# MayDomine/Burst-Attention

Hardware: AMD Instinct MI355X
Metric: attention_fwd_TFLOPs_per_GPU (higher is better)
Workload: dtype fp16; 1 GPU; b=1 seq=262144 h=32 d=128 non-causal; parallelism=ring sequence parallel, sp1

## Files before the change

### burst_attn_amd/build_ext.py

```python

import os
import subprocess
import sys
import sysconfig

PKG_DIR = os.path.dirname(os.path.abspath(__file__))
CSRC = os.path.join(PKG_DIR, "csrc")
BUILD = os.path.join(PKG_DIR, "csrc", "_build")
ARCH = os.environ.get("PYTORCH_ROCM_ARCH", "gfx950")
HIPCC = os.environ.get("HIPCC", "/opt/rocm/bin/hipcc")

DEVICE_SOURCES = ["attn_fwd.hip", "attn_bwd.hip", "probes.hip"]
HOST_SOURCES = ["ext_torch.cpp"]


def _run(cmd, verbose):
    if verbose:
        print("+ " + " ".join(cmd), flush=True)
    r = subprocess.run(cmd, capture_output=True, text=True)
    if r.returncode != 0:
        sys.stderr.write(r.stdout + r.stderr)
        raise RuntimeError(f"build command failed: {' '.join(cmd[:3])} ...")
    return r

# ... 63 lines not shown

def _build_asm_hsaco(verbose, force):
    import json
    import re

    src = os.path.join(CSRC, "attn_fwd.hip")
    s_path = os.path.join(BUILD, "attn_fwd_scaffold.s")
    o_path = os.path.join(BUILD, "attn_fwd_scaffold.o")
    hsaco = os.path.join(PKG_DIR, "_asm_fwd.hsaco")
    syms = os.path.join(PKG_DIR, "_asm_fwd_syms.json")
    patch_mod = os.path.join(PKG_DIR, "..", "tools", "s_patch.py")
    if not (force or _newer(src, hsaco) or _newer(patch_mod, hsaco)):
        return hsaco
    _run([HIPCC, f"--offload-arch={ARCH}", "-O3", "-std=c++17", "-DNDEBUG",
          "-S", "--cuda-device-only", src, "-o", s_path], verbose)
    clang = os.path.join(LLVM, "clang")
    lld = os.path.join(LLVM, "ld.lld")
    _run([clang, "-x", "assembler", "-target", "amdgcn-amd-amdhsa",
          f"-mcpu={ARCH}", "-c", s_path, "-o", o_path], verbose)
    _run([lld, "-shared", o_path, "-o", hsaco], verbose)
    text = open(s_path).read()
    names = {}
    for key, pat in (
        ("f16_accum", r"_ZN12_GLOBAL__N_115attn_fwd_kernelIDF16_Li128ELi64ELi1ELi0ELi1ELi512ELi2ELi0E\S*"),
        ("bf16_accum", r"_ZN12_GLOBAL__N_115attn_fwd_kernelIDF16bLi128ELi64ELi1ELi0ELi1ELi512ELi2ELi0E\S*"),
    ):
        m = re.search(r"\.globl\t(" + pat + ")", text)
        if m:
            names[key] = m.group(1)
    with open(syms, "w") as f:
        json.dump(names, f, indent=1)
    import importlib.util

    spec = importlib.util.spec_from_file_location("s_patch", patch_mod)
    s_patch = importlib.util.module_from_spec(spec)
    spec.loader.exec_module(s_patch)
    sp_path = os.path.join(BUILD, "attn_fwd_patched.s")
    spo_path = os.path.join(BUILD, "attn_fwd_patched.o")
    hsaco_p = os.path.join(PKG_DIR, "_asm_fwd_p.hsaco")
    s_patch.apply("qk_split", s_path, sp_path, list(names.values()))
    _run([clang, "-x", "assembler", "-target", "amdgcn-amd-amdhsa",
          f"-mcpu={ARCH}", "-c", sp_path, "-o", spo_path], verbose)
    _run([lld, "-shared", spo_path, "-o", hsaco_p], verbose)
    if verbose:
        print(f"built {hsaco} and {hsaco_p} (qk_split)")
    return hsaco


# ... 3 lines not shown
```

### burst_attn_amd/csrc/attn_common.h

```cpp
#pragma once
#include <hip/hip_runtime.h>
#include <stdint.h>

typedef __attribute__((ext_vector_type(8))) __bf16 bf16x8_t;
typedef __attribute__((ext_vector_type(8))) _Float16 f16x8_t;
typedef __attribute__((ext_vector_type(16))) float f32x16_t;
typedef __attribute__((ext_vector_type(2))) int i32x2_t;
typedef __attribute__((ext_vector_type(4))) unsigned int u32x4_t;

__device__ __forceinline__ float ba_exp2(float x) {
  return __builtin_amdgcn_exp2f(x);
}

#define BA_LOG2E 1.44269504088896340736f
#define BA_LN2 0.69314718055994530942f
#define BA_NEG_BIG (-1e30f)

template <typename T>
struct mfma_traits;

template <>
struct mfma_traits<_Float16> {
  using frag = f16x8_t;
  static __device__ __forceinline__ f32x16_t mma(frag a, frag b, f32x16_t c) {
// ... 30 lines not shown
template <int SWZ, int SWZ2 = 0>
__device__ __forceinline__ int ba_swz(int byte, int row) {
  return byte ^ ((((row & SWZ) ^ ((row >> 3) & SWZ2))) << 4);
}

template <typename T>
__device__ __forceinline__ void ba_build_frag_pair(
    const f32x16_t& p, typename mfma_traits<T>::frag out[2]) {
  using MT = mfma_traits<T>;
#pragma unroll
  for (int u = 0; u < 2; ++u) {
    unsigned int a0 = MT::pack2(p[8 * u + 0], p[8 * u + 1]);
    unsigned int a1 = MT::pack2(p[8 * u + 2], p[8 * u + 3]);
    unsigned int b0 = MT::pack2(p[8 * u + 4], p[8 * u + 5]);
    unsigned int b1 = MT::pack2(p[8 * u + 6], p[8 * u + 7]);
    i32x2_t r0 = __builtin_amdgcn_permlane32_swap((int)a0, (int)b0, false, false);
    i32x2_t r1 = __builtin_amdgcn_permlane32_swap((int)a1, (int)b1, false, false);
    u32x4_t w = {(unsigned int)r0[0], (unsigned int)r1[0],
                 (unsigned int)r0[1], (unsigned int)r1[1]};
    out[u] = __builtin_bit_cast(typename mfma_traits<T>::frag, w);
  }
}

__device__ __forceinline__ float ba_max16(const f32x16_t& v) {
  float a = fmaxf(fmaxf(v[0], v[1]), v[2]);
  float b = fmaxf(fmaxf(v[3], v[4]), v[5]);
  float c = fmaxf(fmaxf(v[6], v[7]), v[8]);
  float d = fmaxf(fmaxf(v[9], v[10]), v[11]);
  float e = fmaxf(fmaxf(v[12], v[13]), v[14]);
  float f = fmaxf(fmaxf(a, b), v[15]);
  return fmaxf(fmaxf(fmaxf(c, d), e), f);
}

template <typename T, int RS, int SWZ, int SWZ2 = 0>
__device__ __forceinline__ typename mfma_traits<T>::frag ba_ld_rowslice(
    const T* lds, int row, int elem0) {
  int byte = ba_swz<SWZ, SWZ2>(row * (2 * RS) + 2 * elem0, row);
  u32x4_t wv = *(const u32x4_t*)((const char*)lds + byte);
  return __builtin_bit_cast(typename mfma_traits<T>::frag, wv);
}

template <typename T, int RS_T, int SWZ_T, int SWZ2_T = 7>
__device__ __forceinline__ void ba_st_transposed(T* lds, int src_row, int d0,
                                                 const u32x4_t& chunk) {
  const T* e = (const T*)&chunk;
#pragma unroll
// ... 45 lines not shown
```

### burst_attn_amd/csrc/attn_fwd.hip

```cpp

#include "attn_common.h"
#include "attn_host.h"
#include "fwd_variants.h"
#include "gqa_heads.h"

#include <stddef.h>

namespace {

template <int N>
struct ba_ic {
  static constexpr int value = N;
};
struct ba_dyn {
  int value;
};
template <int N>
__device__ __forceinline__ int ba_buf_of(ba_ic<N>) { return N; }
__device__ __forceinline__ int ba_buf_of(ba_dyn d) { return d.value; }

template <typename T, int D, int KVBLK, int OUT_STATE, int VPATH, int SUBT,
          int NT = 512, int NBUF = 2, int KREG = 0>
__global__ __launch_bounds__(NT) void attn_fwd_kernel(
    const T* __restrict__ q, const T* __restrict__ k, const T* __restrict__ v,
    float* __restrict__ o, float* __restrict__ lse,
    int Sq, int Sk, int N, int G,
    int64_t q_sb, int64_t q_ss, int64_t q_sh,
    int64_t k_sb, int64_t k_ss, int64_t k_sh,
    int64_t v_sb, int64_t v_ss, int64_t v_sh,
    float scale, int causal,
    float* __restrict__ st_acc, float* __restrict__ st_m,
    float* __restrict__ st_l,
    int64_t a_sb, int64_t a_ss, int64_t a_sh,
    int64_t ml_sb, int64_t ml_sh, int carry_in) {
  using MT = mfma_traits<T>;
  using frag = typename MT::frag;
  constexpr int SWZ_K = (D == 128) ? 15 : 7;
  constexpr int SWZ_V = 7;
  constexpr int PT = (KVBLK * D / 8) / NT;
  constexpr int QROWS = NT / 2;
  static_assert(PT >= 1, "tile must fill at least one chunk per thread");

  static_assert(KREG != 1 || (SUBT == 1 && NBUF == 2 && VPATH == 0),
                "KREG=1 path: SUBT=1, NBUF=2, V^T image only");
  static_assert(KREG != 2 || (SUBT == 1 && NBUF == 4 && VPATH == 0),
                "KREG=2 path: SUBT=1, NBUF=4 (cross-barrier prefetch)");
  constexpr int IMGS_F = (KREG == 1) ? 1 : 2;
  __shared__ T lds[NBUF * IMGS_F * KVBLK * D];
  auto ldsK = [&](int buf) -> T* { return lds + buf * (IMGS_F * KVBLK * D); };
  auto ldsVT = [&](int buf) -> T* {
    return lds + buf * (IMGS_F * KVBLK * D) + (KREG == 1 ? 0 : KVBLK * D);
  };

  const int tid = threadIdx.x;
  const int lane = tid & 63;
  const int wave = tid >> 6;
  const int l31 = lane & 31;
  const int hi = lane >> 5;
  const int n = blockIdx.y;
  const int b = blockIdx.z;
  const int qb = blockIdx.x * QROWS + wave * 32;
  const int q_row = qb + l31;

  const T* qp = q + (int64_t)b * q_sb + (int64_t)n * q_sh;
  const int nkv = n / G;
  const T* kp = k + (int64_t)b * k_sb + (int64_t)nkv * k_sh;
  const T* vp = v + (int64_t)b * v_sb + (int64_t)nkv * v_sh;

  frag qf[D / 16];
// ... 47 lines not shown
  };
  auto qk_regs = [&](const frag* kf) BA_STEP {
    f32x16_t s = (f32x16_t)(0.f);
#pragma unroll
    for (int i = 0; i < D / 16; ++i) s = MT::mma(kf[i], qf[i], s);
    return s;
  };
  auto qk_lds = [&](int buf, int kvs) BA_STEP {
    f32x16_t s = (f32x16_t)(0.f);
#pragma unroll
    for (int i = 0; i < D / 16; ++i)
      s = MT::mma(k_frag(buf, kvs, i), qf[i], s);
    return s;
  };
  auto mask_sub = [&](f32x16_t& s, int base, int off) BA_STEP {
#pragma unroll
    for (int r = 0; r < 16; ++r) {
      const int kv_g = base + off + ba_crow(r, 0) + 4 * hi;
      if (!(kv_g < Sk && (!causal || kv_g <= q_row))) s[r] = BA_NEG_BIG;
    }
  };
  auto row_max2 = [&](const f32x16_t& s) BA_STEP {
    float tm = ba_max16(s);
    tm = fmaxf(tm, __shfl_xor(tm, 32));
    return tm * c2;
  };
  constexpr float DEFER_THR = 8.f;
  auto rescale = [&](float tm) BA_STEP {
    if (!__all(tm - m2 <= DEFER_THR)) {
      const float mnew = fmaxf(m2, tm);
      const float alpha = ba_exp2(m2 - mnew);
      m2 = mnew;
      lsum *= alpha;
#pragma unroll
      for (int dt = 0; dt < D / 32; ++dt)
#pragma unroll
        for (int r = 0; r < 16; ++r) ot[dt][r] *= alpha;
    }
  };
  auto softmax_tail = [&](f32x16_t& s, float tm, frag* pf) BA_STEP {
    rescale(tm);
    float rowsum = 0.f;
#pragma unroll
    for (int r = 0; r < 16; ++r) {
      s[r] = ba_exp2(__builtin_fmaf(s[r], c2, -m2));
      rowsum += s[r];
    }
    rowsum += __shfl_xor(rowsum, 32);
    lsum += rowsum;
    ba_build_frag_pair<T>(s, pf);
  };
  auto v_frag = [&](int buf, int drow, int kvc) BA_STEP -> frag {
    if (VPATH == 0)
      return ba_ld_rowslice<T, KVBLK, SWZ_V, 7>(ldsVT(buf), drow, kvc + 8 * hi);
    return ba_ld_tr16_frag<T, D>(ldsVT(buf), lane, kvc, drow & ~31);
  };
  auto pv_regs = [&](const frag* vv, const frag* pf) BA_STEP {
#pragma unroll
    for (int dt = 0; dt < D / 32; ++dt)
#pragma unroll
      for (int u = 0; u < 2; ++u)
        ot[dt] = MT::mma(vv[dt * 2 + u], pf[u], ot[dt]);
  };
  struct chunk_rc {
    int row, col8;
  };
  auto stage_rc = [&](int c) BA_STEP {
    const int flat = tid + c * NT;
    return chunk_rc{flat / (D / 8), flat % (D / 8)};
  };
#undef BA_STEP
// ... 39 lines not shown
    if (steady || v_kv0 >= 0) pv_regs(vvP, pvf);
    if (steady || p_kv0 >= 0) {
      softmax_tail(stP, tm, pvf);
      v_kv0 = p_kv0;
      const int kvs_l = (p_kv0 / 32) & 1;
#pragma unroll
      for (int dt = 0; dt < D / 32; ++dt)
#pragma unroll
        for (int u = 0; u < 2; ++u)
          vvP[dt * 2 + u] = v_frag(p_cur, dt * 32 + l31, kvs_l * 32 + 16 * u);
    }
    push_scores(stQ, t * KVBLK + kvs * 32, cur3, full);
  };

  uint32_t k_loff[PT], v_loff[PT];
#pragma unroll
  for (int c = 0; c < PT; ++c) {
    const auto [row, col8] = stage_rc(c);
    k_loff[c] = (uint32_t)((row * k_ss + col8 * 8) * (int64_t)sizeof(T));
    v_loff[c] = (uint32_t)((row * v_ss + col8 * 8) * (int64_t)sizeof(T));
  }
  const bool stage_lin =
      (int64_t)(KVBLK - 1) * k_ss * (int64_t)sizeof(T) + 16 <= 0xffffffffLL &&
      (int64_t)(KVBLK - 1) * v_ss * (int64_t)sizeof(T) + 16 <= 0xffffffffLL;
  auto issue_loads = [&](int tile, u32x4_t* kreg, u32x4_t* vreg) {
    const int kv0 = tile * KVBLK;
    if (SUBT == 1 && stage_lin && kv0 + KVBLK <= Sk) {
      const char* kb = (const char*)(kp + (int64_t)kv0 * k_ss);
      const char* vb = (const char*)(vp + (int64_t)kv0 * v_ss);
#pragma unroll
      for (int c = 0; c < PT; ++c) {
        if (KREG != 1) kreg[c] = *(const u32x4_t*)(kb + k_loff[c]);
        vreg[c] = *(const u32x4_t*)(vb + v_loff[c]);
      }
      return;
    }
#pragma unroll
    for (int c = 0; c < PT; ++c) {
      const auto [row, col8] = stage_rc(c);
      const int kvg = kv0 + row;
      const int kvc = kvg < Sk ? kvg : (Sk - 1);
      if (KREG != 1)
        kreg[c] = *(const u32x4_t*)(kp + (int64_t)kvc * k_ss + col8 * 8);
      vreg[c] = *(const u32x4_t*)(vp + (int64_t)kvc * v_ss + col8 * 8);
    }
  };
  auto write_lds = [&](int buf, const u32x4_t* kreg, const u32x4_t* vreg) {
#pragma unroll
    for (int c = 0; c < PT; ++c) {
      const auto [row, col8] = stage_rc(c);
      if (KREG != 1) {
        const int byte = ba_swz<SWZ_K>(row * (2 * D) + col8 * 16, row);
        *(u32x4_t*)((char*)ldsK(buf) + byte) = kreg[c];
      }
      if (VPATH == 0)
        ba_st_transposed<T, KVBLK, SWZ_V, 7>(ldsVT(buf), row, col8 * 8, vreg[c]);
      else
        ba_st_tr16row<T, D>(ldsVT(buf), row, col8 * 8, vreg[c]);
    }
  };
  auto load_k_sub = [&](int tile, int kvs, frag* dst) {
#pragma unroll
    for (int s = 0; s < D / 16; ++s) {
      const int kvg = tile * KVBLK + kvs * 32 + l31;
      const int kvc = kvg < Sk ? kvg : (Sk - 1);
      dst[s] = __builtin_bit_cast(
          frag, *(const u32x4_t*)(kp + (int64_t)kvc * k_ss + 16 * s + 8 * hi));
    }
  };

  frag kfr[KREG == 1 ? 2 : 1][D / 16];
  {
    u32x4_t kreg[PT], vreg[PT];
    issue_loads(0, kreg, vreg);
    write_lds(0, kreg, vreg);
    if (KREG == 1) {
      load_k_sub(0, 0, kfr[0]);
      load_k_sub(0, 1, kfr[KREG == 1 ? 1 : 0]);
// ... 169 lines not shown
    const float* __restrict__ acc, const float* __restrict__ m,
    const float* __restrict__ l, T* __restrict__ o, float* __restrict__ lse,
    int S, int N) {
  const int lane = threadIdx.x & 63;
  const int wave = threadIdx.x >> 6;
  constexpr int LPR = D / 16;
  const int rows_per_wave = 64 / LPR;
  const int row_in = wave * rows_per_wave + lane / LPR;
  const int sub = lane % LPR;
  const int s = blockIdx.x * 4 * rows_per_wave + row_in;
  const int n = blockIdx.y, b = blockIdx.z;
  if (s >= S) return;
  const float lv = l[((int64_t)b * N + n) * S + s];
  const float inv_l = 1.f / lv;
  const float* arow = acc + (((int64_t)b * S + s) * N + n) * D + sub * 16;
  T* orow = o + (((int64_t)b * S + s) * N + n) * D + sub * 16;
#pragma unroll
  for (int j = 0; j < 16; ++j) orow[j] = (T)(arow[j] * inv_l);
  if (sub == 0)
    lse[((int64_t)b * N + n) * S + s] =
        BA_LN2 * (m[((int64_t)b * N + n) * S + s] + log2f(lv));
}

}

extern "C" const char* bahip_last_error(void) { return ba_g_err; }

struct fwd_args {
  const void *q, *k, *v;
  float *o, *lse;
  int Sq, Sk, N, G;
  int64_t q_sb, q_ss, q_sh, k_sb, k_ss, k_sh, v_sb, v_ss, v_sh;
  float scale;
  int causal;
  float *st_acc, *st_m, *st_l;
  int64_t a_sb, a_ss, a_sh, ml_sb, ml_sh;
  int carry_in;
};

using production_kernel_t = decltype(&attn_fwd_kernel<
    _Float16, 128, 64, 1, BA_FWD_PRODUCTION.vpath, BA_FWD_PRODUCTION.subt,
    BA_FWD_PRODUCTION.nt, BA_FWD_PRODUCTION.nbuf, BA_FWD_PRODUCTION.kreg>);
static_assert(offsetof(fwd_args, carry_in) + sizeof(int) ==
                      kernarg_size<production_kernel_t>::value &&
                  sizeof(fwd_args) ==
                      (kernarg_size<production_kernel_t>::value + 7) / 8 * 8,
              "fwd_args must mirror attn_fwd_kernel's parameter list");

static dim3 fwd_grid(const fwd_args& a, int64_t B, int nt) {
  return dim3((unsigned)((a.Sq + nt / 2 - 1) / (nt / 2)), (unsigned)a.N,
              (unsigned)B);
}

template <typename T, int D, int OUT_STATE, int VPATH, int SUBT, int NT,
          int NBUF, int KREG>
static void launch_fwd(const fwd_args& a, int64_t B, hipStream_t stream) {
  attn_fwd_kernel<T, D, 64, OUT_STATE, VPATH, SUBT, NT, NBUF, KREG>
      <<<fwd_grid(a, B, NT), dim3(NT), 0, stream>>>(
          (const T*)a.q, (const T*)a.k, (const T*)a.v, a.o, a.lse, a.Sq, a.Sk,
          a.N, a.G, a.q_sb, a.q_ss, a.q_sh, a.k_sb, a.k_ss, a.k_sh, a.v_sb, a.v_ss,
          a.v_sh, a.scale, a.causal, a.st_acc, a.st_m, a.st_l, a.a_sb, a.a_ss,
          a.a_sh, a.ml_sb, a.ml_sh, a.carry_in);
}

static int fwd_entry(void* hip_function, int out_state, const void* q,
                     const void* k, const void* v, float* o, float* lse,
                     int64_t B, int64_t Sq, int64_t Sk, int64_t N, int64_t Nk,
                     int64_t D, const int64_t* qs, const int64_t* ks,
                     const int64_t* vs, float scale, int causal, int dtype,
                     float* acc, float* m,
                     float* l, const int64_t* as, const int64_t* mls,
                     int carry_in, void* stream) {
  if (causal && Sq != Sk)
    return ba_fail(BAHIP_ERR_CAUSAL_SHAPE,
                   "causal tiles require Sq == Sk (%d vs %d)", (int)Sq,
                   (int)Sk);
  const int64_t G = ba_gqa_group(N, Nk);
  if (!G)
    return ba_fail(BAHIP_ERR_UNSUPPORTED,
                   "q heads N=%d must be a positive multiple of kv heads "
                   "Nk=%d",
                   (int)N, (int)Nk);
  static const int64_t none[3] = {0, 0, 0};
  if (!out_state) as = mls = none;
  const fwd_args a = {q, k, v, o, lse, (int)Sq, (int)Sk, (int)N, (int)G,
                      qs[0], qs[1], qs[2], ks[0], ks[1], ks[2],
                      vs[0], vs[1], vs[2], scale, causal, acc, m, l,
                      as[0], as[1], as[2], mls[0], mls[1], carry_in};
  if (hip_function) {
    if (D != 128 || (dtype != BAHIP_F16 && dtype != BAHIP_BF16))
      return ba_fail(BAHIP_ERR_UNSUPPORTED,
                     "module forward: unsupported head_dim %d / dtype %d",
                     (int)D, dtype);
    size_t size = sizeof a;
    void* cfg[] = {HIP_LAUNCH_PARAM_BUFFER_POINTER, (void*)&a,
                   HIP_LAUNCH_PARAM_BUFFER_SIZE, &size, HIP_LAUNCH_PARAM_END};
    const dim3 grid = fwd_grid(a, B, BA_FWD_PRODUCTION.nt);
    hipError_t e = hipModuleLaunchKernel(
        (hipFunction_t)hip_function, grid.x, grid.y, grid.z,
        BA_FWD_PRODUCTION.nt, 1, 1, 0, (hipStream_t)stream, nullptr, cfg);
    if (e != hipSuccess)
      return ba_fail((int)e, "module forward launch failed: %s",
                     hipGetErrorString(e));
    return ba_ok();
  }
  ba_fwd_knobs kn;
  kn.vpath = ba_env_int(BA_FWD_KNOB_SPECS[0].env, kn.vpath);
  kn.subt = ba_env_int(BA_FWD_KNOB_SPECS[1].env, kn.subt);
  kn.nt = ba_env_int(BA_FWD_KNOB_SPECS[2].env, kn.nt);
  kn.nbuf = ba_env_int(BA_FWD_KNOB_SPECS[3].env, kn.nbuf);
  kn.kreg = ba_env_int(BA_FWD_KNOB_SPECS[4].env, kn.kreg);
  const ba_fwd_choice c = ba_fwd_select(kn);
  if (c.bad_knob)
    return ba_fail(BAHIP_ERR_BAD_KNOB, "%s=%d is not an accepted value",
                   c.bad_knob, c.bad_value);
  return ba_dispatch_td(D, dtype, [&](auto td) {
    using T = typename decltype(td)::type;
    constexpr int TD = decltype(td)::D;
#define BA_FWD_CASE(VP, ST, NTV, NB, KR)                                   \
  if (c.variant == ba_fwd_variant{VP, ST, NTV, NB, KR}) {                  \
    if (out_state)                                                         \
      launch_fwd<T, TD, 1, VP, ST, NTV, NB, KR>(a, B, (hipStream_t)stream); \
    else                                                                   \
      launch_fwd<T, TD, 0, VP, ST, NTV, NB, KR>(a, B, (hipStream_t)stream); \
  }
    BA_FWD_VARIANTS(BA_FWD_CASE)
#undef BA_FWD_CASE
    return ba_launch_status();
  });
}

extern "C" int bahip_attn_fwd_gqa(
    const void* q, const void* k, const void* v, float* o, float* lse,
    int64_t B, int64_t Sq, int64_t Sk, int64_t N, int64_t Nk, int64_t D,
    const int64_t q_strides[3], const int64_t k_strides[3],
    const int64_t v_strides[3], float softmax_scale, int causal, int dtype,
    void* stream) {
  return fwd_entry(nullptr, 0, q, k, v, o, lse, B, Sq, Sk, N, Nk, D, q_strides,
                   k_strides, v_strides, softmax_scale, causal, dtype, nullptr,
                   nullptr, nullptr, nullptr, nullptr, 0, stream);
}

extern "C" int bahip_attn_fwd_accum_gqa(
    void* hip_function, const void* q, const void* k, const void* v,
    int64_t B, int64_t Sq, int64_t Sk, int64_t N, int64_t Nk, int64_t D,
    const int64_t q_strides[3], const int64_t k_strides[3],
    const int64_t v_strides[3], float softmax_scale, int causal, int dtype,
    float* acc, float* m, float* l, const int64_t acc_strides[3],
    const int64_t ml_strides[2], int carry_in, void* stream) {
  return fwd_entry(hip_function, 1, q, k, v, nullptr, nullptr, B, Sq, Sk, N,
                   Nk, D, q_strides, k_strides, v_strides, softmax_scale,
                   causal, dtype, acc, m, l, acc_strides, ml_strides, carry_in,
                   stream);
}

extern "C" int bahip_attn_fwd(const void* q, const void* k, const void* v,
                              float* o, float* lse, int64_t B, int64_t Sq,
                              int64_t Sk, int64_t N, int64_t D,
                              const int64_t q_strides[3],
                              const int64_t k_strides[3],
                              const int64_t v_strides[3], float softmax_scale,
                              int causal, int dtype, void* stream) {
  return bahip_attn_fwd_gqa(q, k, v, o, lse, B, Sq, Sk, N, N, D, q_strides,
                            k_strides, v_strides, softmax_scale, causal, dtype,
                            stream);
}

extern "C" int bahip_attn_fwd_accum(
    const void* q, const void* k, const void* v, int64_t B, int64_t Sq,
    int64_t Sk, int64_t N, int64_t D, const int64_t q_strides[3],
    const int64_t k_strides[3], const int64_t v_strides[3],
    float softmax_scale, int causal, int dtype, float* acc, float* m,
    float* l, const int64_t acc_strides[3], const int64_t ml_strides[2],
    int carry_in, void* stream) {
  return bahip_attn_fwd_accum_gqa(nullptr, q, k, v, B, Sq, Sk, N, N, D,
                                  q_strides, k_strides, v_strides,
// ... 33 lines not shown
```

### burst_attn_amd/csrc/ext_torch.cpp

```cpp

#include <torch/extension.h>
#include <ATen/hip/HIPContext.h>

#include "../../include/burst_attn_hip.h"
#include "probes.h"

namespace {

int dtype_code(const at::Tensor& t) {
  if (t.scalar_type() == at::kHalf) return BAHIP_F16;
  if (t.scalar_type() == at::kBFloat16) return BAHIP_BF16;
  TORCH_CHECK(false, "burst_attn: expected fp16 or bf16, got ", t.scalar_type());
  return -1;
}

void check_qkv(const at::Tensor& t, const char* name) {
  TORCH_CHECK(t.is_cuda(), name, " must be a GPU tensor");
  TORCH_CHECK(t.dim() == 4, name, " must be [B,S,N,D]");
  TORCH_CHECK(t.stride(3) == 1, name, " head_dim must be contiguous");
  TORCH_CHECK(t.stride(1) % 8 == 0, name,
              " seq stride must be a multiple of 8 elements (16B alignment)");
  TORCH_CHECK(t.stride(2) % 8 == 0, name,
              " head stride must be a multiple of 8 elements");
}
// ... 12 lines not shown
  check_qkv(v, "v");
  TORCH_CHECK(k.size(0) == q.size(0) && v.size(0) == q.size(0),
              "batch mismatch");
  TORCH_CHECK(v.size(2) == k.size(2), "k/v heads mismatch (", k.size(2),
              " vs ", v.size(2), ")");
  TORCH_CHECK(k.size(2) >= 1 && q.size(2) % k.size(2) == 0,
              "heads mismatch: q heads N=", q.size(2),
              " must be a multiple of kv heads Nk=", k.size(2));
  TORCH_CHECK(k.size(3) == q.size(3) && v.size(3) == q.size(3),
              "head_dim mismatch");
  TORCH_CHECK(v.size(1) == k.size(1), "k/v seqlen mismatch");
  TORCH_CHECK(q.scalar_type() == k.scalar_type() &&
                  q.scalar_type() == v.scalar_type(),
              "q/k/v dtype mismatch");
}

#define BA_CALL(expr)                                                      \
  do {                                                                     \
    int rc_ = (expr);                                                      \
    TORCH_CHECK(rc_ == 0, "burst_attn HIP kernel failed (rc=", rc_, "): ", \
                bahip_last_error());                                       \
  } while (0)

std::vector<at::Tensor> attn_fwd(const at::Tensor& q, const at::Tensor& k,
                                 const at::Tensor& v, double softmax_scale,
                                 bool causal) {
  check_qkv3(q, k, v);
  const auto B = q.size(0), Sq = q.size(1), N = q.size(2), D = q.size(3);
  const auto Sk = k.size(1);
  auto o = at::empty({B, Sq, N, D}, q.options().dtype(at::kFloat));
  auto lse = at::empty({B, N, Sq}, q.options().dtype(at::kFloat));
  auto stream = at::hip::getCurrentHIPStream().stream();
  BA_CALL(bahip_attn_fwd_gqa(q.data_ptr(), k.data_ptr(), v.data_ptr(),
                             o.data_ptr<float>(), lse.data_ptr<float>(), B,
                             Sq, Sk, N, k.size(2), D, Strides3(q), Strides3(k),
                             Strides3(v), (float)softmax_scale, causal ? 1 : 0,
                             dtype_code(q), stream));
  return {o, lse};
}

void fwd_accum_call(void* asm_fn, const at::Tensor& q, const at::Tensor& k,
                    const at::Tensor& v, double softmax_scale, bool causal,
                    at::Tensor& acc, at::Tensor& m, at::Tensor& l,
                    bool carry_in) {
  check_qkv3(q, k, v);
  const auto B = q.size(0), Sq = q.size(1), N = q.size(2), D = q.size(3);
  const auto Sk = k.size(1);
  TORCH_CHECK(acc.scalar_type() == at::kFloat && m.scalar_type() == at::kFloat
                  && l.scalar_type() == at::kFloat, "state must be fp32");
  TORCH_CHECK(acc.size(1) == Sq && m.size(2) == Sq && l.size(2) == Sq,
              "state rows must match q rows");
  TORCH_CHECK(acc.stride(3) == 1 && m.stride(2) == 1 && l.stride(2) == 1,
              "state innermost dims must be contiguous");
  int64_t mls[2] = {m.stride(0), m.stride(1)};
  TORCH_CHECK(l.stride(0) == mls[0] && l.stride(1) == mls[1],
              "m/l stride mismatch");
  auto stream = at::hip::getCurrentHIPStream().stream();
  BA_CALL(bahip_attn_fwd_accum_gqa(
      asm_fn, q.data_ptr(), k.data_ptr(), v.data_ptr(), B, Sq, Sk, N,
      k.size(2), D, Strides3(q), Strides3(k), Strides3(v), (float)softmax_scale,
      causal ? 1 : 0, dtype_code(q), acc.data_ptr<float>(),
      m.data_ptr<float>(), l.data_ptr<float>(), Strides3(acc), mls,
      carry_in ? 1 : 0, stream));
}

void attn_fwd_accum(const at::Tensor& q, const at::Tensor& k,
                    const at::Tensor& v, double softmax_scale, bool causal,
                    at::Tensor& acc, at::Tensor& m, at::Tensor& l,
                    bool carry_in) {
  fwd_accum_call(nullptr, q, k, v, softmax_scale, causal, acc, m, l, carry_in);
}

std::vector<at::Tensor> attn_fwd_finalize(const at::Tensor& acc,
                                          const at::Tensor& m,
                                          const at::Tensor& l,
                                          at::ScalarType out_dtype) {
  TORCH_CHECK(acc.is_contiguous() && m.is_contiguous() && l.is_contiguous());
  const auto B = acc.size(0), S = acc.size(1), N = acc.size(2), D = acc.size(3);
  auto o = at::empty({B, S, N, D}, acc.options().dtype(out_dtype));
  auto lse = at::empty({B, N, S}, acc.options().dtype(at::kFloat));
  auto stream = at::hip::getCurrentHIPStream().stream();
  BA_CALL(bahip_attn_fwd_finalize(
      acc.data_ptr<float>(), m.data_ptr<float>(), l.data_ptr<float>(),
      o.data_ptr(), lse.data_ptr<float>(), B, S, N, D,
      out_dtype == at::kHalf ? BAHIP_F16 : BAHIP_BF16, stream));
  return {o, lse};
// ... 121 lines not shown
              b.sizes() == at::IntArrayRef({16, 32}));
  auto d = at::zeros({32, 32}, a.options().dtype(at::kFloat));
  auto stream = at::hip::getCurrentHIPStream().stream();
  BA_CALL(bahip_mfma_probe(a.data_ptr(), b.data_ptr(), d.data_ptr<float>(),
                           dtype_code(a), stream));
  return d;
}

at::Tensor tr16_probe(int64_t mode) {
  auto out = at::zeros({256}, at::TensorOptions().dtype(at::kInt).device(at::kCUDA));
  auto stream = at::hip::getCurrentHIPStream().stream();
  BA_CALL(bahip_tr16_probe((int)mode, out.data_ptr<int>(), stream));
  return out;
}

}

PYBIND11_MODULE(TORCH_EXTENSION_NAME, m) {
  m.def("attn_fwd", &attn_fwd, "BurstAttention fwd tile (gfx950)");
  m.def("attn_fwd_accum", &attn_fwd_accum,
        "carry-in accumulator fwd tile (in-kernel LSE merge)");
  m.def("attn_fwd_finalize", &attn_fwd_finalize,
        "o = acc/l (cast), lse from state");
  m.def("attn_bwd_preprocess", &attn_bwd_preprocess, "delta = rowsum(o*do)",
        py::arg("o"), py::arg("dout"), py::arg("out") = py::none());
  m.def("attn_bwd", &attn_bwd, "BurstAttention bwd tile (gfx950)");
  m.def("attn_bwd_accum", &attn_bwd_accum,
        "bwd tile accumulating into fp32 dq/dk/dv views");
  m.def("mfma_probe", &mfma_probe, "32x32x16 MFMA layout probe");
  m.def("tr16_probe", &tr16_probe, "ds_read_tr16_b64 semantics probe");
  m.def("attn_fwd_asm_load", &attn_fwd_asm_load,
        "load the .s-built forward hsaco (round-3 on-ramp)");
  m.def("attn_fwd_accum_asm", &attn_fwd_accum_asm,
        "carry-in fwd via the hipModule-loaded .s kernel");
}
```

### include/burst_attn_hip.h

```cpp
#pragma once
#include <stdint.h>

#ifdef __cplusplus
extern "C" {
#endif

#define BAHIP_F16 0
#define BAHIP_BF16 1

#define BAHIP_ERR_CAUSAL_SHAPE 1001
#define BAHIP_ERR_UNSUPPORTED 1002
#define BAHIP_ERR_DTYPE_MISMATCH 1003
#define BAHIP_ERR_BAD_KNOB 1004

const char* bahip_last_error(void);

int bahip_attn_fwd(
    const void* q, const void* k, const void* v,
    float* o, float* lse,
    int64_t B, int64_t Sq, int64_t Sk, int64_t N, int64_t D,
    const int64_t q_strides[3],
    const int64_t k_strides[3],
    const int64_t v_strides[3],
    float softmax_scale, int causal, int dtype,
    void* stream);

int bahip_attn_fwd_gqa(
    const void* q, const void* k, const void* v,
    float* o, float* lse,
    int64_t B, int64_t Sq, int64_t Sk, int64_t N, int64_t Nk, int64_t D,
    const int64_t q_strides[3],
    const int64_t k_strides[3],
    const int64_t v_strides[3],
    float softmax_scale, int causal, int dtype,
    void* stream);

// ... 3 lines not shown
    const int64_t q_strides[3], const int64_t k_strides[3],
    const int64_t v_strides[3], float softmax_scale, int causal, int dtype,
    float* acc, float* m, float* l, const int64_t acc_strides[3],
    const int64_t ml_strides[2], int carry_in, void* stream);

int bahip_attn_fwd_accum_fn(
    void* hip_function,
    const void* q, const void* k, const void* v,
    int64_t B, int64_t Sq, int64_t Sk, int64_t N, int64_t D,
    const int64_t q_strides[3], const int64_t k_strides[3],
    const int64_t v_strides[3], float softmax_scale, int causal, int dtype,
    float* acc, float* m, float* l, const int64_t acc_strides[3],
    const int64_t ml_strides[2], int carry_in, void* stream);

int bahip_attn_fwd_accum_gqa(
    void* hip_function,
    const void* q, const void* k, const void* v,
    int64_t B, int64_t Sq, int64_t Sk, int64_t N, int64_t Nk, int64_t D,
    const int64_t q_strides[3], const int64_t k_strides[3],
    const int64_t v_strides[3], float softmax_scale, int causal, int dtype,
    float* acc, float* m, float* l, const int64_t acc_strides[3],
    const int64_t ml_strides[2], int carry_in, void* stream);

int bahip_attn_fwd_finalize(
    const float* acc, const float* m, const float* l, void* o, float* lse,
    int64_t B, int64_t S, int64_t N, int64_t D, int dtype, void* stream);

int bahip_attn_bwd_preprocess(
    const void* o, const void* dout, float* delta,
    int64_t B, int64_t S, int64_t N, int64_t D,
    const int64_t o_strides[3], const int64_t do_strides[3],
    int o_dtype, int do_dtype, void* stream);

int bahip_attn_bwd(
    const void* dout, const void* q, const void* k, const void* v,
    const float* delta, const float* lse,
    float* dq, float* dk, float* dv,
    int64_t B, int64_t Sq, int64_t Sk, int64_t N, int64_t D,
    const int64_t do_strides[3], const int64_t q_strides[3],
    const int64_t k_strides[3], const int64_t v_strides[3],
    const int64_t delta_strides[2], const int64_t lse_strides[2],
    const int64_t dq_strides[3], const int64_t dk_strides[3],
    const int64_t dv_strides[3],
    float softmax_scale, int causal, int deterministic, int dtype,
    void* stream);

// ... 17 lines not shown
```

Measured before the change: 978.0 TFLOP/s/GPU.

## Pre-transpose V into a tiled V^T image and read it directly in forward

Adds a pre-pass kernel that writes V as a blocked, pre-transposed V^T image in a workspace. The forward kernel then loads that image with plain b128 copies into LDS instead of running a per-element transposing store every tile. It also swaps the cross-half row max/sum shuffles for permlane32_swap on the V^T path. The change is auto-enabled when Q-tile reuse (Sq/256*G) is at least 16. The cost is an extra kernel launch, a full extra read and write of V, and a workspace allocation on each call.

After: 1025 TFLOP/s/GPU (median of 6 runs). 4.8% higher.

```diff
diff --git a/burst_attn_amd/build_ext.py b/burst_attn_amd/build_ext.py
--- a/burst_attn_amd/build_ext.py
+++ b/burst_attn_amd/build_ext.py
@@ -109,8 +109,8 @@
     text = open(s_path).read()
     names = {}
     for key, pat in (
-        ("f16_accum", r"_ZN12_GLOBAL__N_115attn_fwd_kernelIDF16_Li128ELi64ELi1ELi0ELi1ELi512ELi2ELi0E\S*"),
-        ("bf16_accum", r"_ZN12_GLOBAL__N_115attn_fwd_kernelIDF16bLi128ELi64ELi1ELi0ELi1ELi512ELi2ELi0E\S*"),
+        ("f16_accum", r"_ZN12_GLOBAL__N_115attn_fwd_kernelIDF16_Li128ELi64ELi1ELi0ELi1ELi512ELi2ELi0ELi0EE\S*"),
+        ("bf16_accum", r"_ZN12_GLOBAL__N_115attn_fwd_kernelIDF16bLi128ELi64ELi1ELi0ELi1ELi512ELi2ELi0ELi0EE\S*"),
     ):
         m = re.search(r"\.globl\t(" + pat + ")", text)
         if m:
diff --git a/burst_attn_amd/csrc/attn_common.h b/burst_attn_amd/csrc/attn_common.h
--- a/burst_attn_amd/csrc/attn_common.h
+++ b/burst_attn_amd/csrc/attn_common.h
@@ -76,6 +76,13 @@
   }
 }
 
+__device__ __forceinline__ void ba_half_pair(float x, float& lo, float& hi) {
+  const int xi = __builtin_bit_cast(int, x);
+  const i32x2_t r = __builtin_amdgcn_permlane32_swap(xi, xi, false, false);
+  lo = __builtin_bit_cast(float, (int)r[0]);
+  hi = __builtin_bit_cast(float, (int)r[1]);
+}
+
 __device__ __forceinline__ float ba_max16(const f32x16_t& v) {
   float a = fmaxf(fmaxf(v[0], v[1]), v[2]);
   float b = fmaxf(fmaxf(v[3], v[4]), v[5]);
diff --git a/burst_attn_amd/csrc/attn_fwd.hip b/burst_attn_amd/csrc/attn_fwd.hip
--- a/burst_attn_amd/csrc/attn_fwd.hip
+++ b/burst_attn_amd/csrc/attn_fwd.hip
@@ -3,6 +3,7 @@
 #include "attn_host.h"
 #include "fwd_variants.h"
 #include "gqa_heads.h"
+#include "vt_image.h"
 
 #include <stddef.h>
 
@@ -20,7 +21,7 @@
 __device__ __forceinline__ int ba_buf_of(ba_dyn d) { return d.value; }
 
 template <typename T, int D, int KVBLK, int OUT_STATE, int VPATH, int SUBT,
-          int NT = 512, int NBUF = 2, int KREG = 0>
+          int NT = 512, int NBUF = 2, int KREG = 0, int VSRC = 0>
 __global__ __launch_bounds__(NT) void attn_fwd_kernel(
     const T* __restrict__ q, const T* __restrict__ k, const T* __restrict__ v,
     float* __restrict__ o, float* __restrict__ lse,
@@ -39,12 +40,16 @@
   constexpr int SWZ_V = 7;
   constexpr int PT = (KVBLK * D / 8) / NT;
   constexpr int QROWS = NT / 2;
+  constexpr bool HSWAP = VSRC == 1;
   static_assert(PT >= 1, "tile must fill at least one chunk per thread");
 
   static_assert(KREG != 1 || (SUBT == 1 && NBUF == 2 && VPATH == 0),
                 "KREG=1 path: SUBT=1, NBUF=2, V^T image only");
   static_assert(KREG != 2 || (SUBT == 1 && NBUF == 4 && VPATH == 0),
                 "KREG=2 path: SUBT=1, NBUF=4 (cross-barrier prefetch)");
+  static_assert(VSRC == 0 || (VPATH == 0 && SUBT == 1 && KREG == 0 &&
+                              KVBLK == BA_VT_KVBLK),
+                "the V^T image source: b128-read V^T LDS image, SUBT=1");
   constexpr int IMGS_F = (KREG == 1) ? 1 : 2;
   __shared__ T lds[NBUF * IMGS_F * KVBLK * D];
   auto ldsK = [&](int buf) -> T* { return lds + buf * (IMGS_F * KVBLK * D); };
@@ -138,7 +143,13 @@
   };
   auto row_max2 = [&](const f32x16_t& s) BA_STEP {
     float tm = ba_max16(s);
-    tm = fmaxf(tm, __shfl_xor(tm, 32));
+    if (HSWAP) {
+      float lo, hi2;
+      ba_half_pair(tm, lo, hi2);
+      tm = fmaxf(lo, hi2);
+    } else {
+      tm = fmaxf(tm, __shfl_xor(tm, 32));
+    }
     return tm * c2;
   };
   constexpr float DEFER_THR = 8.f;
@@ -162,7 +173,13 @@
       s[r] = ba_exp2(__builtin_fmaf(s[r], c2, -m2));
       rowsum += s[r];
     }
-    rowsum += __shfl_xor(rowsum, 32);
+    if (HSWAP) {
+      float lo, hi2;
+      ba_half_pair(rowsum, lo, hi2);
+      rowsum = lo + hi2;
+    } else {
+      rowsum += __shfl_xor(rowsum, 32);
+    }
     lsum += rowsum;
     ba_build_frag_pair<T>(s, pf);
   };
@@ -248,16 +265,23 @@
   }
   const bool stage_lin =
       (int64_t)(KVBLK - 1) * k_ss * (int64_t)sizeof(T) + 16 <= 0xffffffffLL &&
-      (int64_t)(KVBLK - 1) * v_ss * (int64_t)sizeof(T) + 16 <= 0xffffffffLL;
+      (VSRC == 1 ||
+       (int64_t)(KVBLK - 1) * v_ss * (int64_t)sizeof(T) + 16 <= 0xffffffffLL);
   auto issue_loads = [&](int tile, u32x4_t* kreg, u32x4_t* vreg) {
     const int kv0 = tile * KVBLK;
+    if (VSRC == 1) {
+      const char* vb = (const char*)(vp + tile * ba_vt_block_elems(D));
+#pragma unroll
+      for (int c = 0; c < PT; ++c)
+        vreg[c] = *(const u32x4_t*)(vb + (uint32_t)((tid + c * NT) * 16));
+    }
     if (SUBT == 1 && stage_lin && kv0 + KVBLK <= Sk) {
       const char* kb = (const char*)(kp + (int64_t)kv0 * k_ss);
       const char* vb = (const char*)(vp + (int64_t)kv0 * v_ss);
 #pragma unroll
       for (int c = 0; c < PT; ++c) {
         if (KREG != 1) kreg[c] = *(const u32x4_t*)(kb + k_loff[c]);
-        vreg[c] = *(const u32x4_t*)(vb + v_loff[c]);
+        if (VSRC == 0) vreg[c] = *(const u32x4_t*)(vb + v_loff[c]);
       }
       return;
     }
@@ -268,7 +292,8 @@
       const int kvc = kvg < Sk ? kvg : (Sk - 1);
       if (KREG != 1)
         kreg[c] = *(const u32x4_t*)(kp + (int64_t)kvc * k_ss + col8 * 8);
-      vreg[c] = *(const u32x4_t*)(vp + (int64_t)kvc * v_ss + col8 * 8);
+      if (VSRC == 0)
+        vreg[c] = *(const u32x4_t*)(vp + (int64_t)kvc * v_ss + col8 * 8);
     }
   };
   auto write_lds = [&](int buf, const u32x4_t* kreg, const u32x4_t* vreg) {
@@ -279,7 +304,11 @@
         const int byte = ba_swz<SWZ_K>(row * (2 * D) + col8 * 16, row);
         *(u32x4_t*)((char*)ldsK(buf) + byte) = kreg[c];
       }
-      if (VPATH == 0)
+      if (VSRC == 1) {
+        const int flat = tid + c * NT;
+        const int byte = ba_swz<SWZ_V, 7>(flat * 16, flat / (KVBLK / 8));
+        *(u32x4_t*)((char*)ldsVT(buf) + byte) = vreg[c];
+      } else if (VPATH == 0)
         ba_st_transposed<T, KVBLK, SWZ_V, 7>(ldsVT(buf), row, col8 * 8, vreg[c]);
       else
         ba_st_tr16row<T, D>(ldsVT(buf), row, col8 * 8, vreg[c]);
@@ -495,6 +524,39 @@
         BA_LN2 * (m[((int64_t)b * N + n) * S + s] + log2f(lv));
 }
 
+template <typename T, int D>
+__global__ __launch_bounds__(256) void attn_vt_image_kernel(
+    const T* __restrict__ v, T* __restrict__ img, int Sk, int Nk,
+    int64_t v_sb, int64_t v_ss, int64_t v_sh, int64_t img_elems) {
+  constexpr int KVBLK = BA_VT_KVBLK;
+  constexpr int NT = 256;
+  constexpr int PT = (KVBLK * D / 8) / NT;
+  __shared__ T lds[KVBLK * D];
+  const int tid = threadIdx.x;
+  const int t = blockIdx.x, nkv = blockIdx.y, b = blockIdx.z;
+  const T* vp = v + (int64_t)b * v_sb + (int64_t)nkv * v_sh;
+#pragma unroll
+  for (int c = 0; c < PT; ++c) {
+    const int flat = tid + c * NT;
+    const int row = flat / (D / 8), col8 = flat % (D / 8);
+    const int kvg = t * KVBLK + row;
+    u32x4_t chunk = {0, 0, 0, 0};
+    if (kvg < Sk)
+      chunk = *(const u32x4_t*)(vp + (int64_t)kvg * v_ss + col8 * 8);
+    ba_st_transposed<T, KVBLK, 7, 7>(lds, row, col8 * 8, chunk);
+  }
+  __syncthreads();
+  const int64_t blk = ba_vt_offset(Nk, Sk, D, b, nkv, (int64_t)t * KVBLK, 0);
+#pragma unroll
+  for (int c = 0; c < PT; ++c) {
+    const int flat = tid + c * NT;
+    const auto f = ba_ld_rowslice<T, KVBLK, 7, 7>(lds, flat / (KVBLK / 8),
+                                                  (flat % (KVBLK / 8)) * 8);
+    const int64_t e = blk + (int64_t)flat * 8;
+    if (e + 8 <= img_elems) *(u32x4_t*)(img + e) = __builtin_bit_cast(u32x4_t, f);
+  }
+}
+
 }
 
 extern "C" const char* bahip_last_error(void) { return ba_g_err; }
@@ -526,14 +588,59 @@
 }
 
 template <typename T, int D, int OUT_STATE, int VPATH, int SUBT, int NT,
-          int NBUF, int KREG>
+          int NBUF, int KREG, int VSRC = 0>
 static void launch_fwd(const fwd_args& a, int64_t B, hipStream_t stream) {
-  attn_fwd_kernel<T, D, 64, OUT_STATE, VPATH, SUBT, NT, NBUF, KREG>
+  attn_fwd_kernel<T, D, 64, OUT_STATE, VPATH, SUBT, NT, NBUF, KREG, VSRC>
       <<<fwd_grid(a, B, NT), dim3(NT), 0, stream>>>(
           (const T*)a.q, (const T*)a.k, (const T*)a.v, a.o, a.lse, a.Sq, a.Sk,
           a.N, a.G, a.q_sb, a.q_ss, a.q_sh, a.k_sb, a.k_ss, a.k_sh, a.v_sb, a.v_ss,
           a.v_sh, a.scale, a.causal, a.st_acc, a.st_m, a.st_l, a.a_sb, a.a_ss,
           a.a_sh, a.ml_sb, a.ml_sh, a.carry_in);
+}
+
+static int fwd_read_knobs(int64_t Sq, int64_t G, ba_fwd_choice* c,
+                          bool* use_vt) {
+  ba_fwd_knobs kn;
+  kn.vpath = ba_env_int(BA_FWD_KNOB_SPECS[0].env, kn.vpath);
+  kn.subt = ba_env_int(BA_FWD_KNOB_SPECS[1].env, kn.subt);
+  kn.nt = ba_env_int(BA_FWD_KNOB_SPECS[2].env, kn.nt);
+  kn.nbuf = ba_env_int(BA_FWD_KNOB_SPECS[3].env, kn.nbuf);
+  kn.kreg = ba_env_int(BA_FWD_KNOB_SPECS[4].env, kn.kreg);
+  *c = ba_fwd_select(kn);
+  if (c->bad_knob)
+    return ba_fail(BAHIP_ERR_BAD_KNOB, "%s=%d is not an accepted value",
+                   c->bad_knob, c->bad_value);
+  const char* e = getenv("BA_FWD_VT");
+  const int vt = e ? e[0] - '0' : -1;
+  if (e && !((vt == 0 || vt == 1) && e[1] == '\0'))
+    return ba_fail(BAHIP_ERR_BAD_KNOB, "BA_FWD_VT=%s is not an accepted value",
+                   e);
+  *use_vt = c->variant == BA_FWD_PRODUCTION &&
+            (vt < 0 ? ba_vt_reuse(Sq, G) >= BA_VT_AUTO_MIN_REUSE : vt == 1);
+  return 0;
+}
+
+static int vt_image_entry(const void* v, void* img, int64_t img_bytes,
+                          int64_t B, int64_t Sk, int64_t Nk, int64_t D,
+                          const int64_t* vs, int dtype, void* stream) {
+  if (B < 1 || Sk < 1 || Nk < 1 || Nk > 65535 || B > 65535)
+    return ba_fail(BAHIP_ERR_UNSUPPORTED,
+                   "V^T image: unsupported shape B=%d Sk=%d Nk=%d", (int)B,
+                   (int)Sk, (int)Nk);
+  if (!img || !ba_vt_workspace_fits(img_bytes, B, Nk, Sk, D))
+    return ba_fail(BAHIP_ERR_WORKSPACE,
+                   "V^T image workspace of %lld bytes is smaller than the "
+                   "%lld needed",
+                   (long long)img_bytes, (long long)ba_vt_bytes(B, Nk, Sk, D));
+  const dim3 grid((unsigned)ba_vt_tiles(Sk), (unsigned)Nk, (unsigned)B);
+  return ba_dispatch_td(D, dtype, [&](auto td) {
+    using T = typename decltype(td)::type;
+    attn_vt_image_kernel<T, decltype(td)::D>
+        <<<grid, 256, 0, (hipStream_t)stream>>>(
+            (const T*)v, (T*)img, (int)Sk, (int)Nk, vs[0], vs[1], vs[2],
+            img_bytes / (int64_t)sizeof(T));
+    return ba_launch_status();
+  });
 }
 
 static int fwd_entry(void* hip_function, int out_state, const void* q,
@@ -543,7 +650,7 @@
                      const int64_t* vs, float scale, int causal, int dtype,
                      float* acc, float* m,
                      float* l, const int64_t* as, const int64_t* mls,
-                     int carry_in, void* stream) {
+                     int carry_in, void* ws, int64_t ws_bytes, void* stream) {
   if (causal && Sq != Sk)
     return ba_fail(BAHIP_ERR_CAUSAL_SHAPE,
                    "causal tiles require Sq == Sk (%d vs %d)", (int)Sq,
@@ -577,16 +684,31 @@
                      hipGetErrorString(e));
     return ba_ok();
   }
-  ba_fwd_knobs kn;
-  kn.vpath = ba_env_int(BA_FWD_KNOB_SPECS[0].env, kn.vpath);
-  kn.subt = ba_env_int(BA_FWD_KNOB_SPECS[1].env, kn.subt);
-  kn.nt = ba_env_int(BA_FWD_KNOB_SPECS[2].env, kn.nt);
-  kn.nbuf = ba_env_int(BA_FWD_KNOB_SPECS[3].env, kn.nbuf);
-  kn.kreg = ba_env_int(BA_FWD_KNOB_SPECS[4].env, kn.kreg);
-  const ba_fwd_choice c = ba_fwd_select(kn);
-  if (c.bad_knob)
-    return ba_fail(BAHIP_ERR_BAD_KNOB, "%s=%d is not an accepted value",
-                   c.bad_knob, c.bad_value);
+  ba_fwd_choice c;
+  bool use_vt;
+  if (int rc = fwd_read_knobs(Sq, G, &c, &use_vt)) return rc;
+  if (use_vt && ws) {
+    if (int rc = vt_image_entry(v, ws, ws_bytes, B, Sk, Nk, D, vs, dtype,
+                                stream))
+      return rc;
+    fwd_args ai = a;
+    ai.v = ws;
+    ai.v_sb = ba_vt_batch_stride(Nk, Sk, D);
+    ai.v_ss = 0;
+    ai.v_sh = ba_vt_head_stride(Sk, D);
+    return ba_dispatch_td(D, dtype, [&](auto td) {
+      using T = typename decltype(td)::type;
+      constexpr int TD = decltype(td)::D;
+      constexpr ba_fwd_variant P = BA_FWD_PRODUCTION;
+      if (out_state)
+        launch_fwd<T, TD, 1, P.vpath, P.subt, P.nt, P.nbuf, P.kreg, 1>(
+            ai, B, (hipStream_t)stream);
+      else
+        launch_fwd<T, TD, 0, P.vpath, P.subt, P.nt, P.nbuf, P.kreg, 1>(
+            ai, B, (hipStream_t)stream);
+      return ba_launch_status();
+    });
+  }
   return ba_dispatch_td(D, dtype, [&](auto td) {
     using T = typename decltype(td)::type;
     constexpr int TD = decltype(td)::D;
@@ -611,7 +733,57 @@
     void* stream) {
   return fwd_entry(nullptr, 0, q, k, v, o, lse, B, Sq, Sk, N, Nk, D, q_strides,
                    k_strides, v_strides, softmax_scale, causal, dtype, nullptr,
-                   nullptr, nullptr, nullptr, nullptr, 0, stream);
+                   nullptr, nullptr, nullptr, nullptr, 0, nullptr, 0, stream);
+}
+
+extern "C" int bahip_attn_fwd_gqa_ws(
+    const void* q, const void* k, const void* v, float* o, float* lse,
+    int64_t B, int64_t Sq, int64_t Sk, int64_t N, int64_t Nk, int64_t D,
+    const int64_t q_strides[3], const int64_t k_strides[3],
+    const int64_t v_strides[3], float softmax_scale, int causal, int dtype,
+    void* workspace, int64_t workspace_bytes, void* stream) {
+  return fwd_entry(nullptr, 0, q, k, v, o, lse, B, Sq, Sk, N, Nk, D, q_strides,
+                   k_strides, v_strides, softmax_scale, causal, dtype, nullptr,
+                   nullptr, nullptr, nullptr, nullptr, 0, workspace,
+                   workspace_bytes, stream);
+}
+
+extern "C" int bahip_attn_fwd_accum_gqa_ws(
+    void* hip_function, const void* q, const void* k, const void* v,
+    int64_t B, int64_t Sq, int64_t Sk, int64_t N, int64_t Nk, int64_t D,
+    const int64_t q_strides[3], const int64_t k_strides[3],
+    const int64_t v_strides[3], float softmax_scale, int causal, int dtype,
+    float* acc, float* m, float* l, const int64_t acc_strides[3],
+    const int64_t ml_strides[2], int carry_in, void* workspace,
+    int64_t workspace_bytes, void* stream) {
+  return fwd_entry(hip_function, 1, q, k, v, nullptr, nullptr, B, Sq, Sk, N,
+                   Nk, D, q_strides, k_strides, v_strides, softmax_scale,
+                   causal, dtype, acc, m, l, acc_strides, ml_strides, carry_in,
+                   workspace, workspace_bytes, stream);
+}
+
+extern "C" int64_t bahip_attn_vt_image_bytes(int64_t B, int64_t Nk,
+                                             int64_t Sk, int64_t D) {
+  return ba_vt_bytes(B, Nk, Sk, D);
+}
+
+extern "C" int64_t bahip_attn_fwd_workspace_bytes(int64_t B, int64_t Sq,
+                                                  int64_t Sk, int64_t N,
+                                                  int64_t Nk, int64_t D) {
+  ba_fwd_choice c;
+  bool use_vt;
+  const int64_t G = ba_gqa_group(N, Nk);
+  if (!G || fwd_read_knobs(Sq, G, &c, &use_vt) || !use_vt) return 0;
+  return ba_vt_bytes(B, Nk, Sk, D);
+}
+
+extern "C" int bahip_attn_vt_image(const void* v, void* image,
+                                   int64_t image_bytes, int64_t B, int64_t Sk,
+                                   int64_t Nk, int64_t D,
+                                   const int64_t v_strides[3], int dtype,
+                                   void* stream) {
+  return vt_image_entry(v, image, image_bytes, B, Sk, Nk, D, v_strides, dtype,
+                        stream);
 }
 
 extern "C" int bahip_attn_fwd_accum_gqa(
@@ -624,7 +796,7 @@
   return fwd_entry(hip_function, 1, q, k, v, nullptr, nullptr, B, Sq, Sk, N,
                    Nk, D, q_strides, k_strides, v_strides, softmax_scale,
                    causal, dtype, acc, m, l, acc_strides, ml_strides, carry_in,
-                   stream);
+                   nullptr, 0, stream);
 }
 
 extern "C" int bahip_attn_fwd(const void* q, const void* k, const void* v,
diff --git a/burst_attn_amd/csrc/ext_torch.cpp b/burst_attn_amd/csrc/ext_torch.cpp
--- a/burst_attn_amd/csrc/ext_torch.cpp
+++ b/burst_attn_amd/csrc/ext_torch.cpp
@@ -58,6 +58,13 @@
                 bahip_last_error());                                       \
   } while (0)
 
+at::Tensor fwd_workspace(const at::Tensor& q, const at::Tensor& k) {
+  const int64_t bytes = bahip_attn_fwd_workspace_bytes(
+      q.size(0), q.size(1), k.size(1), q.size(2), k.size(2), q.size(3));
+  if (bytes <= 0) return at::Tensor();
+  return at::empty({bytes}, q.options().dtype(at::kByte));
+}
+
 std::vector<at::Tensor> attn_fwd(const at::Tensor& q, const at::Tensor& k,
                                  const at::Tensor& v, double softmax_scale,
                                  bool causal) {
@@ -66,13 +73,40 @@
   const auto Sk = k.size(1);
   auto o = at::empty({B, Sq, N, D}, q.options().dtype(at::kFloat));
   auto lse = at::empty({B, N, Sq}, q.options().dtype(at::kFloat));
-  auto stream = at::hip::getCurrentHIPStream().stream();
-  BA_CALL(bahip_attn_fwd_gqa(q.data_ptr(), k.data_ptr(), v.data_ptr(),
-                             o.data_ptr<float>(), lse.data_ptr<float>(), B,
-                             Sq, Sk, N, k.size(2), D, Strides3(q), Strides3(k),
-                             Strides3(v), (float)softmax_scale, causal ? 1 : 0,
-                             dtype_code(q), stream));
+  auto ws = fwd_workspace(q, k);
+  auto stream = at::hip::getCurrentHIPStream().stream();
+  BA_CALL(bahip_attn_fwd_gqa_ws(
+      q.data_ptr(), k.data_ptr(), v.data_ptr(), o.data_ptr<float>(),
+      lse.data_ptr<float>(), B, Sq, Sk, N, k.size(2), D, Strides3(q),
+      Strides3(k), Strides3(v), (float)softmax_scale, causal ? 1 : 0,
+      dtype_code(q), ws.defined() ? ws.data_ptr() : nullptr,
+      ws.defined() ? ws.numel() : 0, stream));
   return {o, lse};
+}
+
+at::Tensor attn_vt_image(const at::Tensor& v, c10::optional<at::Tensor> out) {
+  check_qkv(v, "v");
+  const auto B = v.size(0), Sk = v.size(1), Nk = v.size(2), D = v.size(3);
+  const int64_t T = (Sk + 63) / 64;
+  at::Tensor img;
+  if (out.has_value()) {
+    img = *out;
+    TORCH_CHECK(img.is_cuda() && img.scalar_type() == v.scalar_type() &&
+                    img.is_contiguous() &&
+                    (img.dim() == 1 ||
+                     img.sizes() == at::IntArrayRef({B, Nk, T, D, 64})),
+                "image out must be contiguous, of v's dtype, and either "
+                "[B,Nk,ceil(Sk/64),D,64] or a flat workspace");
+  } else {
+    img = at::empty({B, Nk, T, D, 64}, v.options());
+  }
+  auto stream = at::hip::getCurrentHIPStream().stream();
+  BA_CALL(bahip_attn_vt_image(v.data_ptr(), img.data_ptr(),
+                              img.numel() * img.element_size(), B, Sk, Nk, D,
+                              Strides3(v), dtype_code(v), stream));
+  if (img.dim() == 1) return img.narrow(0, 0, B * Nk * T * D * 64)
+                          .view({B, Nk, T, D, 64});
+  return img;
 }
 
 void fwd_accum_call(void* asm_fn, const at::Tensor& q, const at::Tensor& k,
@@ -91,13 +125,15 @@
   int64_t mls[2] = {m.stride(0), m.stride(1)};
   TORCH_CHECK(l.stride(0) == mls[0] && l.stride(1) == mls[1],
               "m/l stride mismatch");
-  auto stream = at::hip::getCurrentHIPStream().stream();
-  BA_CALL(bahip_attn_fwd_accum_gqa(
+  auto ws = asm_fn ? at::Tensor() : fwd_workspace(q, k);
+  auto stream = at::hip::getCurrentHIPStream().stream();
+  BA_CALL(bahip_attn_fwd_accum_gqa_ws(
       asm_fn, q.data_ptr(), k.data_ptr(), v.data_ptr(), B, Sq, Sk, N,
       k.size(2), D, Strides3(q), Strides3(k), Strides3(v), (float)softmax_scale,
       causal ? 1 : 0, dtype_code(q), acc.data_ptr<float>(),
       m.data_ptr<float>(), l.data_ptr<float>(), Strides3(acc), mls,
-      carry_in ? 1 : 0, stream));
+      carry_in ? 1 : 0, ws.defined() ? ws.data_ptr() : nullptr,
+      ws.defined() ? ws.numel() : 0, stream));
 }
 
 void attn_fwd_accum(const at::Tensor& q, const at::Tensor& k,
@@ -265,6 +301,12 @@
         "carry-in accumulator fwd tile (in-kernel LSE merge)");
   m.def("attn_fwd_finalize", &attn_fwd_finalize,
         "o = acc/l (cast), lse from state");
+  m.def("attn_vt_image", &attn_vt_image,
+        "V^T image [B,Nk,ceil(Sk/64),D,64] the forward's pre-pass writes",
+        py::arg("v"), py::arg("out") = py::none());
+  m.def("attn_fwd_workspace_bytes", &bahip_attn_fwd_workspace_bytes,
+        "V^T image bytes a forward of (B, Sq, Sk, N, Nk, D) allocates under "
+        "the current knobs; 0 = in-kernel transpose");
   m.def("attn_bwd_preprocess", &attn_bwd_preprocess, "delta = rowsum(o*do)",
         py::arg("o"), py::arg("dout"), py::arg("out") = py::none());
   m.def("attn_bwd", &attn_bwd, "BurstAttention bwd tile (gfx950)");
diff --git a/burst_attn_amd/csrc/vt_image.h b/burst_attn_amd/csrc/vt_image.h
--- /dev/null
+++ b/burst_attn_amd/csrc/vt_image.h
@@ -0,0 +1,35 @@
+#pragma once
+#include <stdint.h>
+
+constexpr int BA_VT_KVBLK = 64;
+
+constexpr int64_t ba_vt_tiles(int64_t Sk) {
+  return (Sk + BA_VT_KVBLK - 1) / BA_VT_KVBLK;
+}
+constexpr int64_t ba_vt_block_elems(int64_t D) { return D * BA_VT_KVBLK; }
+constexpr int64_t ba_vt_head_stride(int64_t Sk, int64_t D) {
+  return ba_vt_tiles(Sk) * ba_vt_block_elems(D);
+}
+constexpr int64_t ba_vt_batch_stride(int64_t Nk, int64_t Sk, int64_t D) {
+  return Nk * ba_vt_head_stride(Sk, D);
+}
+constexpr int64_t ba_vt_bytes(int64_t B, int64_t Nk, int64_t Sk, int64_t D,
+                              int64_t elem_bytes = 2) {
+  return B * ba_vt_batch_stride(Nk, Sk, D) * elem_bytes;
+}
+constexpr bool ba_vt_workspace_fits(int64_t ws_bytes, int64_t B, int64_t Nk,
+                                    int64_t Sk, int64_t D,
+                                    int64_t elem_bytes = 2) {
+  return ws_bytes >= ba_vt_bytes(B, Nk, Sk, D, elem_bytes);
+}
+constexpr int64_t ba_vt_offset(int64_t Nk, int64_t Sk, int64_t D, int64_t b,
+                               int64_t nkv, int64_t kv, int64_t d) {
+  return b * ba_vt_batch_stride(Nk, Sk, D) + nkv * ba_vt_head_stride(Sk, D) +
+         (kv / BA_VT_KVBLK) * ba_vt_block_elems(D) + d * BA_VT_KVBLK +
+         kv % BA_VT_KVBLK;
+}
+
+constexpr int64_t BA_VT_AUTO_MIN_REUSE = 16;
+constexpr int64_t ba_vt_reuse(int64_t Sq, int64_t G) {
+  return (Sq + 255) / 256 * G;
+}
diff --git a/include/burst_attn_hip.h b/include/burst_attn_hip.h
--- a/include/burst_attn_hip.h
+++ b/include/burst_attn_hip.h
@@ -12,6 +12,7 @@
 #define BAHIP_ERR_UNSUPPORTED 1002
 #define BAHIP_ERR_DTYPE_MISMATCH 1003
 #define BAHIP_ERR_BAD_KNOB 1004
+#define BAHIP_ERR_WORKSPACE 1005
 
 const char* bahip_last_error(void);
 
@@ -61,6 +62,33 @@
     float* acc, float* m, float* l, const int64_t acc_strides[3],
     const int64_t ml_strides[2], int carry_in, void* stream);
 
+int64_t bahip_attn_vt_image_bytes(int64_t B, int64_t Nk, int64_t Sk,
+                                  int64_t D);
+int64_t bahip_attn_fwd_workspace_bytes(int64_t B, int64_t Sq, int64_t Sk,
+                                       int64_t N, int64_t Nk, int64_t D);
+int bahip_attn_vt_image(
+    const void* v, void* image, int64_t image_bytes,
+    int64_t B, int64_t Sk, int64_t Nk, int64_t D,
+    const int64_t v_strides[3], int dtype, void* stream);
+int bahip_attn_fwd_gqa_ws(
+    const void* q, const void* k, const void* v,
+    float* o, float* lse,
+    int64_t B, int64_t Sq, int64_t Sk, int64_t N, int64_t Nk, int64_t D,
+    const int64_t q_strides[3],
+    const int64_t k_strides[3],
+    const int64_t v_strides[3],
+    float softmax_scale, int causal, int dtype,
+    void* workspace, int64_t workspace_bytes, void* stream);
+int bahip_attn_fwd_accum_gqa_ws(
+    void* hip_function,
+    const void* q, const void* k, const void* v,
+    int64_t B, int64_t Sq, int64_t Sk, int64_t N, int64_t Nk, int64_t D,
+    const int64_t q_strides[3], const int64_t k_strides[3],
+    const int64_t v_strides[3], float softmax_scale, int causal, int dtype,
+    float* acc, float* m, float* l, const int64_t acc_strides[3],
+    const int64_t ml_strides[2], int carry_in,
+    void* workspace, int64_t workspace_bytes, void* stream);
+
 int bahip_attn_fwd_finalize(
     const float* acc, const float* m, const float* l, void* o, float* lse,
     int64_t B, int64_t S, int64_t N, int64_t D, int dtype, void* stream);
```
